# arpg/ba

Measured on AMD Instinct MI355X. Metric: Gauss-Newton iterations/sec, higher is better.
Workload: dtype f64; 1 GPU; BASELINE.json configs[3]: 10000 poses / 1000000 landmarks / 10000000 reprojection residuals, pinhole, LmSize=1, PoseSize=6, Gauss-Newton (no dogleg), 2 anchor poses inactive; poses=10000, landmarks=1000000, residuals=10000000, reduced_system_n=59988, driver=phase calls of the C-ABI (include/ba_hip.h), parallelism=single GPU

## Files before the change

ba_amd/csrc/chol_kernels.h:

```cpp
#pragma once
#include "engine.h"

namespace bae {

void launch_panel_chain(const CholSwitches& sw, hipStream_t s, double* dA, uint32_t ld, uint32_t nblk, uint32_t J,
                        uint32_t Jend, double* dsgn, double* opbuf, int* colneg, int* flags, const uint8_t* nz,
                        const uint32_t* rl = nullptr, uint32_t rl_n = 0, bool rl_square = false, bool sq = false);
void launch_step_update(hipStream_t s, dim3 grid, double* dA, uint32_t ld, uint32_t nblk, uint32_t c0, uint32_t kb0,
                        uint32_t kb1, double* dsgn, double* opbuf, int* colneg, int* flags, const uint8_t* nz,
                        const uint32_t* rl);
void launch_rect128(const CholSwitches& sw, const Rect128Shape& r, hipStream_t s, double* dA, uint32_t ld, uint32_t nblk,
                    uint32_t c0, uint32_t ncols, uint32_t kb0, uint32_t kb1, const double* dsgn, const int* colneg,
                    const uint8_t* nz, const OwnMap& own);
void launch_bulk_update(const CholSwitches& sw, Engine* e, hipStream_t s, double* dA, uint32_t ld, uint32_t nblk,
                        uint32_t a_end, uint32_t J, uint32_t Jend, const double* dsgn, const int* colneg,
                        const uint8_t* nz, bool full, const OwnMap& own, const uint2* pairs = nullptr,
                        uint32_t npairs = 0);
void launch_linvT(hipStream_t s, uint32_t nblk, const double* opbuf, const double* dsgn, double* linvT);
void launch_backward(hipStream_t s, double* dA, uint32_t ld, uint32_t nblk, const double* linvT, double* dx,
                     const uint8_t* nz, uint32_t lo = 0, uint32_t hi = 0xffffffffu);
int setup_status_block(Engine* e, const double* dA, uint32_t ld, hipStream_t s0);

}
```

ba_amd/csrc/chol_launch.h:

```cpp
#pragma once
#include <stdint.h>
#include <stdlib.h>
#include <string.h>

#include <algorithm>

namespace bae {

static const uint32_t kTile = 64;
static const uint32_t kPacketStride = 40 * 64;
static const uint32_t kKin = 4;

struct CholSwitches {
  bool no128 = false;
  bool no_lookahead = false;
  bool bulk_full = false;
  bool dense = false;
  bool no_dist_solve = false;
  uint32_t sbl = 3;
  uint32_t rect_min_rows = 128;
  uint32_t bulk_full_m = 128;
  bool c_rmw = false;
  uint32_t kout = 4;
  uint32_t left_min_tiles = 512;
  bool square = false;
  uint32_t sq_w = kKin;
  const char* dist_layout = nullptr;
  bool dense_scatter = false;
  const char* trace_file = nullptr;
};

inline uint32_t parse_kout(const char* v, uint32_t nblk) {
  const uint32_t k = v ? (uint32_t)atoi(v) : 0;
  return k ? k : (nblk >= 400 ? 16u : nblk >= 256 ? 8u : 4u);
}
inline void parse_process_switches(CholSwitches* sw, const char* no128, const char* no_lookahead, const char* bulk_full,
                                   const char* dense, const char* no_dist_solve, const char* sbl,
                                   const char* bulk_full_m, const char* c_rmw = nullptr) {
  sw->no128 = no128 != nullptr;
  sw->no_lookahead = no_lookahead != nullptr;
  sw->bulk_full = bulk_full != nullptr;
  sw->dense = dense != nullptr;
  sw->no_dist_solve = no_dist_solve != nullptr;
  sw->sbl = sbl ? (uint32_t)atoi(sbl) : 3u;
  sw->rect_min_rows = bulk_full_m ? (uint32_t)std::max(16, atoi(bulk_full_m)) : 128u;
  sw->bulk_full_m = bulk_full_m ? (uint32_t)atoi(bulk_full_m) : 128u;
  sw->c_rmw = c_rmw != nullptr;
}
inline void parse_call_switches(CholSwitches* sw, uint32_t nblk, const char* kout, const char* left_min_tiles,
                                const char* square, const char* sq_w, const char* dist_layout,
                                const char* dense_scatter, const char* trace_file) {
  sw->kout = parse_kout(kout, nblk);
  sw->left_min_tiles = left_min_tiles ? (uint32_t)std::max(1, atoi(left_min_tiles)) : 512u;
  sw->square = nblk < 512 && square && atoi(square) != 0;
  sw->sq_w = sq_w ? std::min(4u, std::max(1u, (uint32_t)atoi(sq_w))) : kKin;
  sw->dist_layout = dist_layout;
  sw->dense_scatter = dense_scatter != nullptr;
  sw->trace_file = trace_file;
}

inline const CholSwitches& chol_process_switches() {
  static const CholSwitches once = [] {
    CholSwitches sw;
    parse_process_switches(&sw, getenv("BA_HIP_NO128"), getenv("BA_HIP_NO_LOOKAHEAD"), getenv("BA_HIP_BULK_FULL"),
                           getenv("BA_HIP_DENSE"), getenv("BA_HIP_NO_DIST_SOLVE"), getenv("BA_HIP_SBL"),
                           getenv("BA_HIP_BULK_FULL_M"), getenv("BA_HIP_C_RMW"));
    return sw;
  }();
  return once;
}
inline CholSwitches chol_switches(uint32_t nblk) {
  CholSwitches sw = chol_process_switches();
  parse_call_switches(&sw, nblk, getenv("BA_HIP_KOUT"), getenv("BA_HIP_LEFT_MIN_TILES"), getenv("BA_HIP_SQUARE"),
                      getenv("BA_HIP_SQ_W"), getenv("BA_HIP_DIST_LAYOUT"), getenv("BA_HIP_DENSE_SCATTER"),
                      getenv("BA_HIP_TRACE_FILE"));
  return sw;
}
inline uint32_t kout_from_env(uint32_t nblk) { return parse_kout(getenv("BA_HIP_KOUT"), nblk); }

struct ChainShape { bool left; uint32_t kin; };
inline ChainShape chain_shape(uint32_t nblk, const CholSwitches& sw) {
  const bool left = nblk >= sw.left_min_tiles;
  return {left, left ? 2 * kKin : kKin};
}

struct Rect128Shape { bool use128; uint32_t m2, rect_cols, nrow64, grid; };
enum RectRule { kRectSingle, kRectDist };
inline Rect128Shape rect128_shape(RectRule rule, uint32_t nblk, uint32_t c0, uint32_t ncols, uint32_t G,
                                  const CholSwitches& sw) {
  const uint32_t r0 = c0 + ncols, m = nblk - r0;
  const bool single = r0 + sw.rect_min_rows <= nblk;
  const bool dist = m >= 16 && G % 2u == 0;
  Rect128Shape r = {!sw.no128 && (rule == kRectSingle ? single : dist) && ncols % 2u == 0 && c0 % 2u == 0, 0, 0, 0, 0};
  if (!r.use128) return r;
  r.m2 = m / 2;
  r.rect_cols = ncols / 2;
  r.nrow64 = (ncols * (1 + (m & 1u)) + 7) / 8 * 8;
  r.grid = r.nrow64 + r.m2 * r.rect_cols;
  return r;
}

enum BulkKernel { kBulkU128, kBulkU128List, kBulkU2Full, kBulkU2Capped };
struct BulkShape { BulkKernel kernel; uint32_t grid, nrow64, m2, sbl; int swzf; };
inline BulkShape bulk_shape(uint32_t nblk, uint32_t a_end, bool full, uint32_t own_n, uint32_t own_G, bool have_pairs,
                            uint32_t npairs, const CholSwitches& sw) {
  const uint32_t m = nblk - a_end;
  if (full && !sw.no128 && m >= 16 && (a_end % 2u) == 0 && (own_n <= 1 || own_G % 2u == 0)) {
    const uint32_t m2 = m / 2, sbl2 = 2, sbe2 = 1u << sbl2;
    const uint32_t nsr = (m2 + sbe2 - 1) / sbe2, nsb = nsr * (nsr + 1) / 2;
    const uint32_t nrow64 = (m * (1 + (m & 1u)) + 7) / 8 * 8;
    if (have_pairs && own_n > 1 && a_end % own_G == 0)
      return {kBulkU128List, nrow64 + npairs * (own_G / 2) * (own_G / 2), nrow64, m2, sbl2, 0};
    return {kBulkU128, nrow64 + ((nsb + 7) / 8) * 8 * sbe2 * sbe2, nrow64, m2, sbl2, 0};
  }
  const uint32_t sbe = 1u << sw.sbl;
  const uint32_t nsr = (m + 1 + sbe - 1) / sbe, nsb = nsr * (nsr + 1) / 2;
  return {full ? kBulkU2Full : kBulkU2Capped, ((nsb + 7) / 8) * 8 * sbe * sbe, 0, 0, sw.sbl, 1 | (int)(sw.sbl << 8)};
}

struct FactorWork {
  size_t dsgn, linvT, opbuf, colneg, total;
  explicit FactorWork(uint32_t nblk)
      : dsgn(0), linvT((size_t)nblk * kTile), opbuf(linvT + (size_t)nblk * kTile * kTile),
        colneg(opbuf + (size_t)nblk * kPacketStride), total(colneg + (nblk + 1) / 2) {}
};

inline uint64_t dist_plan_key(uint64_t nzL_version, uint32_t kout, bool pat, const char* layout, bool dense_scatter) {
  static const char* const names[] = {"auto", "tri", "grid", "col", "row"};
  uint64_t lay = layout && *layout ? 5 : 0;
  for (uint64_t i = 0; i < 5 && lay == 5; ++i)
    if (!strcmp(layout, names[i])) lay = i;
  return (pat ? nzL_version : 0) << 24 | (uint64_t)std::min(kout, 0xffffu) << 8 | lay << 2 |
         (dense_scatter ? 2u : 0u) | (pat ? 1u : 0u);
}

}
```

ba_amd/csrc/engine.h:

```cpp
#pragma once
#include <hip/hip_runtime.h>
#include <stdint.h>
#include <atomic>
#include <string>
#include <utility>
#include <vector>

#include "../../include/ba_hip.h"
#include "structure.h"
#include "ordering.h"
#include "selinv.h"
#include "marg.h"
#include "pcg.h"
#include "dist_plan.h"
#include "lifecycle.h"
#include "chol_launch.h"

namespace bae {

inline std::atomic<int64_t> g_device_bytes_live{0};
template <typename T>
struct DBuf {
  T* p = nullptr;
  size_t n = 0;
  DBuf() = default;
  DBuf(const DBuf&) = delete;
  DBuf& operator=(const DBuf&) = delete;
  DBuf(DBuf&& o) noexcept : p(o.p), n(o.n) { o.p = nullptr; o.n = 0; }
  DBuf& operator=(DBuf&& o) noexcept {
    if (this != &o) { release(); p = o.p; n = o.n; o.p = nullptr; o.n = 0; }
    return *this;
  }
  ~DBuf() { release(); }
  hipError_t alloc(size_t count) {
    if (count <= n && p) return hipSuccess;
    release();
    if (count == 0) { n = 0; return hipSuccess; }
    hipError_t err = hipMalloc((void**)&p, count * sizeof(T));
    if (err == hipSuccess) { n = count; g_device_bytes_live += (int64_t)bytes(); }
    return err;
  }
  void release() {
    if (p) { (void)hipFree(p); g_device_bytes_live -= (int64_t)bytes(); }
    p = nullptr;
    n = 0;
  }
  size_t bytes() const { return n * sizeof(T); }
};

static const int kRt = 12;
static const int kCamRec = 37;
static const int kPoseState = 16;
static const int kRow = 6;

struct Structure : Lists {
  uint32_t n_pp_entries = 0;
};

struct Engine {
  int lm_dim = 1, pose_dim = 6, device = 0;
  int calib_dim = 0;
  bool calib_tvs = false;
  std::vector<double> cam_params_prev;
  std::vector<double> cam_w_prev;
  bool has_fov = false;
  DBuf<double> lm_zref;
  hipStream_t stream = nullptr;
  hipStream_t stream2 = nullptr;
  std::vector<hipEvent_t> ev_panel, ev_bulk;
  hipEvent_t ev_imu_start = nullptr, ev_imu_done = nullptr;
  hipEvent_t ev_fork = nullptr, ev_join = nullptr;
  bool imu_early_pending = false;
  bool own_stream = false;
  std::string err;
  ba_hip_options opt;
  Problem prob;
  Structure st;
  Held held;
  int cur = 0;
  ba_hip_timers timers;
// ... 19 lines not shown
  DBuf<double> pose_cam;
  const double* pose_cam_ptr() const { return prob.pose_cam_params.empty() ? nullptr : pose_cam.p; }
  DBuf<int32_t> pose_opt, lm_opt;
  DBuf<uint16_t> pose_mask;
  DBuf<uint16_t> pose_mask_lin;
  uint64_t mask_version = 0, lin_mask_version = 0;
  const uint16_t* lin_pose_mask() const { return mask_version == lin_mask_version ? pose_mask.p : pose_mask_lin.p; }
  DBuf<uint32_t> lm_ref_pose, lm_ref_cam;
  DBuf<uint32_t> lm_ptr;
  DBuf<double> obs_z;
  DBuf<uint32_t> obs_pose, obs_cam, obs_lm, obs_rid;
  DBuf<double> obs_w0;
  DBuf<uint8_t> obs_cond;
  DBuf<uint2> wave_rng;
  DBuf<uint32_t> tile_ptr;
  DBuf<uint2> tile_ref;
  DBuf<uint32_t> tile_order;
  DBuf<uint4> tile_desc;
  uint32_t n_tile_order = 0;
  uint64_t tile_order_version = ~0ull;
  uint64_t tile_order_plan = ~0ull;
  int dbg_assemble_variant = 5;
  int dbg_host_structure = 0;
  int dbg_linearize_variant = 0;
  int dbg_tile_order = 0;
  int dbg_imu_wave = -1;
  int dbg_all_tiles = 0;
  DBuf<uint2> pair_ent;
  DBuf<uint32_t> pose_ptr, pose_mid;
  DBuf<uint32_t> pose_ent;
  DBuf<uint8_t> nzL;
  std::vector<uint8_t> nzL_host;
  uint64_t nzL_version = 0;
  std::vector<uint8_t> nzS_host;
  struct Dist {
    uint64_t key = ~0ull;
    DistPlan plan;
    DistTables tab;
    DBuf<uint32_t> tiles;
    DBuf<uint2> pairs;
    DBuf<uint32_t> square_rows;
    DBuf<uint32_t> dense_rows;
    DBuf<uint4> send_rects, recv_rects;
    DBuf<double> msg;
    DBuf<double> usend, urecv;
    DBuf<double> ssend, srecv;
    DBuf<double> back;
    hipStream_t stream3 = nullptr;
    hipStream_t stream4 = nullptr;
    void* comm2 = nullptr;
    std::vector<hipEvent_t> ev;
  } dist;
  void sharding_changed() { held.sharding_changed(); dist.key = ~0ull; }
  std::string dist_layout_name;
  ba_hip_comm_stats cstats = {};
  DBuf<double> packed;

  DBuf<uint8_t> pose_active;
  DBuf<uint32_t> un_pose; DBuf<double> un_t, un_cov_inv, un_scale; DBuf<uint8_t> un_rot;
  DBuf<uint32_t> bin_p1, bin_p2; DBuf<double> bin_t, bin_cov_inv, bin_cov_inv_sqrt, bin_w;
  DBuf<uint8_t> bin_rot;
  DBuf<uint32_t> imu_p1, imu_p2, imu_ptr; DBuf<double> imu_meas, imu_consts, imu_cov_inv;
  bool imu_cov_once = false;
  DBuf<double> imu_frozen;
  DBuf<double> imu_steps;
  DBuf<uint8_t> imu_cov_done;
// ... 220 lines not shown
int launch_end_solve(Engine* e);
int launch_residual_vectors(Engine* e, double* d_r2);
int launch_residuals(Engine* e, int mode);
int launch_landmarks(Engine* e, double c_huber, int use_robust);
int launch_gather_S(Engine* e);
int launch_pack_lower(Engine* e, int unpack);
size_t packed_lower_count(uint32_t n_pad);
int launch_backsub(Engine* e);
int launch_compose_step(Engine* e, double coef_rhs, double coef_gn, double* norms2_host);
int launch_apply_step(Engine* e);
int launch_dogleg(Engine* e, int gn_available, double* h7, bool skip_jrhs);
int select_kth(Engine* e, const double* d_values, uint32_t n_local, uint64_t k, double* out);
int sum_partials(Engine* e, uint32_t nparts, uint32_t ncomp, double* host_out, bool cross_shard = true);
void defer_begin(Engine* e);
int defer_flush(Engine* e);
struct DeferScope {
  Engine* e;
  bool flushed = false;
  explicit DeferScope(Engine* eng) : e(eng) { defer_begin(e); }
  DeferScope(const DeferScope&) = delete;
  DeferScope& operator=(const DeferScope&) = delete;
  int flush() { flushed = true; return defer_flush(e); }
  ~DeferScope() {
    if (flushed) return;
    e->defer_active = false;
    e->defer_n = 0;
  }
};
int launch_imu_early(Engine* e, double c_huber_proj);
int launch_posepose_build(Engine* e, double c_huber_proj, double* h3);
int launch_posepose_eval(Engine* e, double* h3);
int launch_posepose_jrhs(Engine* e, double* out);
int cholesky_solve(Engine* e, double* dA, uint32_t n, uint32_t ld, double* dx, int* status,
                   const uint8_t* nz_tiles);
int factor_tile_pattern(Engine* e);
uint32_t choose_kout(uint32_t nblk);
bool dist_solve_enabled(const Engine* e);
int dist_reduce_scatter_S(Engine* e);
int launch_imu_residual_vectors(Engine* e, double* d_r15);
int build_tile_order(Engine* e);
int build_tile_desc(Engine* e);
int dist_assembly_tiles(Engine* e, std::vector<uint8_t>* need);
int build_lists_device(Engine* e, const std::function<void(const char*)>& stage);
int order_poses(Engine* e, std::vector<uint64_t>* proj_edges, double device_ms);
bool ordering_wants_graph(const Engine* e);
int dist_broadcast(Engine* e, double* buf, size_t count, int root, hipStream_t s);
struct DistXfer { double* buf; size_t count; int peer; bool send; };
int dist_exchange(Engine* e, const std::vector<DistXfer>& x, bool side, hipStream_t s);
int dist_allreduce_stream(Engine* e, double* buf, size_t count, hipStream_t s);
void comm_release(Engine* e);
int check_solve_residual(Engine* e, const double* dS, const double* dx, const double* db, double* out2);
int cholesky_solve_dist(Engine* e, double* dA, uint32_t ld, double* dx, int* status, const uint8_t* nz);
int trailing_marginals(Engine* e, const double* dA, uint32_t ld, uint32_t first, uint32_t K, double* cov);
int marginals_compute(Engine* e);
int marginals_gather(Engine* e, uint32_t n, const std::vector<uint32_t>& ra, const std::vector<uint32_t>& rb, int Da,
                     int Db, double* out);
int marginals_landmarks(Engine* e, uint32_t n, const uint32_t* ids, double* out);
void marginals_release(Engine* e);
int leverages_run(Engine* e, uint32_t n, const uint32_t* ids, double* out);
int pose_pose_leverages_run(Engine* e, int kind, uint32_t n, const uint32_t* ids, double* cov, double* info, double* lev);
int jointcov_run(Engine* e, const std::vector<uint32_t>& sel, const std::vector<uint32_t>& lms, double* out);
void jointcov_release(Engine* e);
struct JointPlan;
struct SubstTables {
  const uint4 *chunks, *rows;
  const uint32_t *src, *pos;
};
// ... 34 lines not shown
```

ba_amd/csrc/engine.hip:

```cpp
#include "entry.h"
#include <chrono>
#include <functional>
#include <memory>
#include <thread>

#include <algorithm>
#include <cmath>
#include <cstdlib>
#include <cstring>
#include <numeric>

#include "dmath.h"
#include "factorsolve.h"
#include "dpose.h"

namespace bae {

int Engine::fail(hipError_t e, const char* what) {
  err = std::string(what) + ": " + hipGetErrorString(e);
  return -(int)(e == hipSuccess ? 1 : e);
}
void Engine::prof_collect() {
  auto drain = [](std::vector<std::pair<hipEvent_t, hipEvent_t>>& v, double& ms, uint32_t& n) {
    for (auto& p : v) {
// ... 972 lines not shown
    if (!e->held.nzL_valid && (rc = factor_tile_pattern(e))) return rc;
    const bool rebuild = e->pcg_plan_version != e->nzL_version || e->pcg_plan.nt != st.ld / 64 || e->pcg_blk.size() != (size_t)2 * st.ld;
    if (rebuild) {
      build_pcg_plan(e->nzS_host, st.ld / 64, e->pcg_plan);
      pcg_row_blocks(st.np, (uint32_t)e->pose_dim, st.K, st.ld, e->pcg_blk, e->pcg_blocks);
      e->pcg_plan_version = e->nzL_version;
      e->pcg_coarse_built = 0;
    }
    if (e->pcg_opt.coarse_aggregate && e->pcg_coarse_built != e->pcg_opt.coarse_aggregate) {
      const uint32_t D = (uint32_t)e->pose_dim;
      std::vector<uint32_t> nat(st.ld, kPcgNone);
      uint32_t a = 0;
      for (uint32_t p = 0; p < st.P; ++p)
        if (st.pose_opt[p] >= 0) {
          for (uint32_t d = 0; d < D; ++d) nat[(size_t)st.pose_opt[p] * D + d] = a * D + d;
          ++a;
        }
      for (uint32_t k = 0; k < st.K; ++k) nat[st.np + k] = st.Pact * D + k;
      build_pcg_coarse(e->pcg_plan, nat, st.Pact, D, st.K, e->pcg_opt.coarse_aggregate);
      e->pcg_coarse_built = e->pcg_opt.coarse_aggregate;
    }
    if ((rc = pcg_solve_device(e, e->A.p, st.n, st.ld, e->rhs_sc.p, e->pcg_plan, e->nzS_host, e->pcg_blk, e->pcg_blocks, rebuild,
                               e->pcg_opt, e->gn_p.p, &e->pcg_stats, &status))) return rc;
    e->held.solved_by_pcg();
  } else if (st.n > 0 && !skip) {
    if (e->opt.keep_reduced_system) {
      BAE_HIP(e->A_keep.alloc((size_t)st.ld * st.ld));
      BAE_HIP(hipMemcpyAsync(e->A_keep.p, e->A.p, (size_t)st.ld * st.ld * sizeof(double),
                             hipMemcpyDeviceToDevice, e->stream));
    }
    if (!e->held.nzL_valid && (rc = factor_tile_pattern(e))) return rc;
    if (dist_solve_enabled(e)) {
      if ((rc = cholesky_solve_dist(e, e->A.p, st.ld, e->gn_p.p, &status, e->nzL.p))) return rc;
    } else if ((rc = cholesky_solve(e, e->A.p, st.n, st.ld, e->gn_p.p, &status, e->nzL.p))) return rc;
    e->held.solved_directly();
  }
  e->timers.solve = t.stop_ms();
  EventTimer tb(e);
  if ((rc = launch_backsub(e))) return rc;
  e->timers.back_substitution = tb.stop_ms();
  return status ? BA_HIP_FACTORIZATION_ERROR : 0;
}

int ba_hip_dogleg_terms(ba_hip_engine* h, int gn_available, ba_hip_dogleg_scalars* out) {
  BA_ENTRY_FINAL(h);
  memset(out, 0, sizeof(*out));
  double* dh = e->dog_h;
  const bool reuse = gn_available && e->held.dog_jrhs_valid;
  DeferScope sums(e);
  int rc = launch_dogleg(e, gn_available, dh, reuse);
  if (!rc && !reuse) rc = launch_posepose_jrhs(e, dh + 7);
  if (!rc && !reuse) rc = launch_priors_jrhs(e, &e->prior_jrhs_h);
  if (!rc) rc = sums.flush();
  e->held.dogleg_sums(!rc);
  if (rc) return rc;
  out->rhs_p_sq = dh[0]; out->gn_p_sq = dh[1]; out->rhs_gn_p = dh[2];
  out->rhs_l_sq = dh[3]; out->gn_l_sq = dh[4]; out->rhs_gn_l = dh[5];
  out->j_rhs_sq = dh[6] + dh[7] + e->prior_jrhs_h;
  return e->st.K ? launch_calib_dogleg(e, gn_available, out) : 0;
}

int ba_hip_compose_step(ba_hip_engine* h, double coef_rhs, double coef_gn, ba_hip_step_norms* out) {
  BA_ENTRY_FINAL(h);
  double n2[2];
  DeferScope sums(e);
  int rc = launch_compose_step(e, coef_rhs, coef_gn, n2);
  if (!rc) rc = sums.flush();
// ... 369 lines not shown
```

ba_amd/csrc/engine_readers.hip:

```cpp
#include <algorithm>
#include <cmath>
#include <cstring>

#include "entry.h"
#include "factorsolve.h"

namespace bae {

static_assert(kRequestMaxBlock == kPcgMaxBlock, "block_ok of requests.h states the limit of pcg.h");

struct PaddedSystem {
  uint32_t ld = 0, nt = 0;
  std::vector<double> A;
  std::vector<uint8_t> nz;
};
static PaddedSystem pad_system(uint32_t n, const double* a_lower, const double* b, bool want_nz) {
  PaddedSystem s;
  const uint32_t ld = s.ld = std::max(((n + 63) / 64) * 64, 64u), nt = s.nt = ld / 64;
  s.A.assign((size_t)(ld + 1) * ld, 0.0);
  if (want_nz) s.nz.assign((size_t)nt * nt, 0);
  for (uint32_t r = 0; r < n; ++r)
    for (uint32_t c = 0; c <= r; ++c) {
      const double v = a_lower[(size_t)r * n + c];
      s.A[(size_t)r * ld + c] = v;
// ... 661 lines not shown
  const int rc = pcg_panel_solve_device(e, dA.p, n, ld, plan, sys.nz, blk, blocks, identity_rowmap(n, ld).data(), m, B, X, *o, &status);
  if (rc) return rc;
  e->held.pcg_run_finished(false);
  if (stats) *stats = e->pcgp_stats;
  return status ? BA_HIP_FACTORIZATION_ERROR : 0;
}

static int tile_factorise(Engine* e, const char* who, uint32_t n, const double* a_lower, const double* b,
                          const uint8_t* tile_map, PaddedSystem& sys, DBuf<double>& dA, DBuf<double>& dx, int* status) {
  sys = pad_system(n, a_lower, b, true);
  const uint32_t ld = sys.ld, nt = sys.nt;
  std::vector<uint8_t>& nz = sys.nz;
  if (tile_map) {
    for (uint32_t r = 0; r < n; ++r)
      for (uint32_t c = 0; c <= r; ++c)
        if (a_lower[(size_t)r * n + c] != 0.0 && r / 64 != c / 64 && !tile_map[(size_t)(r / 64) * nt + c / 64]) {
          e->err = std::string(who) + ": entry (" + std::to_string(r) + ", " + std::to_string(c) + ") is nonzero but tile (" +
                   std::to_string(r / 64) + ", " + std::to_string(c / 64) + ") is not in the tile map";
          return -1;
        }
    for (uint32_t i = 0; i < nt; ++i)
      for (uint32_t k = 0; k <= i; ++k) nz[(size_t)i * nt + k] |= tile_map[(size_t)i * nt + k] ? 1 : 0;
  }
  for (uint32_t i = 0; i < nt; ++i) nz[(size_t)i * nt + i] = 1;
  tile_symbolic_factor(nz, nt);
  DBuf<uint8_t> dnz;
  BAE_HIP(dA.alloc(sys.A.size()));
  BAE_HIP(dx.alloc(ld));
  BAE_HIP(dnz.alloc(nz.size()));
  BAE_HIP(e->flags.alloc(16));
  BAE_HIP(hipMemcpy(dA.p, sys.A.data(), sys.A.size() * 8, hipMemcpyHostToDevice));
  BAE_HIP(hipMemcpy(dnz.p, nz.data(), nz.size(), hipMemcpyHostToDevice));
  e->held.standalone_factorisation();
  int rc = cholesky_solve(e, dA.p, n, ld, dx.p, status, dnz.p);
  if (rc) return rc;
  BAE_HIP(hipDeviceSynchronize());
  return 0;
}
int ba_hip_tile_solve(ba_hip_engine* h, uint32_t n, const double* a_lower, const double* b, const uint8_t* tile_map,
                      double* x, uint8_t* nz_factor, double* factor, double* linvT, double* dsgn) {
  BA_ENTRY_DEVICE(h);
  if (!n || !a_lower || !b || !x) return e->fail_msg("ba_hip_tile_solve: NULL or empty argument");
  PaddedSystem sys;
  DBuf<double> dA, dx;
  int status = 0;
  if (int rc = tile_factorise(e, "ba_hip_tile_solve", n, a_lower, b, tile_map, sys, dA, dx, &status)) return rc;
  const uint32_t ld = sys.ld, nt = sys.nt;
  if (nz_factor) std::copy(sys.nz.begin(), sys.nz.end(), nz_factor);
  hipError_t err = download_x(dx, n, x);
  if (err == hipSuccess && factor) err = hipMemcpy(factor, dA.p, (size_t)ld * ld * 8, hipMemcpyDeviceToHost);
  const FactorWork fw(nt);
  if (err == hipSuccess && dsgn) err = hipMemcpy(dsgn, e->invdiag.p + fw.dsgn, (size_t)ld * 8, hipMemcpyDeviceToHost);
  if (err == hipSuccess && linvT)
    err = hipMemcpy(linvT, e->invdiag.p + fw.linvT, (size_t)nt * 64 * 64 * 8, hipMemcpyDeviceToHost);
  if (err != hipSuccess) return e->fail(err, "hipMemcpy");
  return status ? BA_HIP_FACTORIZATION_ERROR : 0;
}

int ba_hip_tile_factor_solve(ba_hip_engine* h, uint32_t n, const double* a_lower, const uint8_t* tile_map, uint32_t m,
                             const double* B, double* X) {
  BA_ENTRY_DEVICE(h);
  static const char* what = "ba_hip_tile_factor_solve";
  if (!n || !a_lower) return e->fail_msg("ba_hip_tile_factor_solve: NULL or empty argument");
  BA_ASK(columns_ok(what, m, BA_HIP_FACTOR_SOLVE_MAX_COLUMNS, "BA_HIP_FACTOR_SOLVE_MAX_COLUMNS"));
  if (!B || !X) return e->fail_msg("ba_hip_tile_factor_solve: NULL argument");
  PaddedSystem sys;
  DBuf<double> dA, dx;
// ... 11 lines not shown
```

ba_amd/csrc/hostcheck.cpp:

```cpp
#include <vector>
#include "dmath.h"
using namespace bad;

static Rt rt_from7(const double* p) {
  Rt t;
  t.R = quat_to_rot(p[3], p[4], p[5], p[6]);
  t.t = v3(p[0], p[1], p[2]);
  return t;
}

static double g_hostcheck_fov_w = 0.0;
extern "C" void ba_hostcheck_set_fov(double w) { g_hostcheck_fov_w = w; }
static Cam cam_from4(const double* cam4) {
  Cam c = {cam4[0], cam4[1], cam4[2], cam4[3], g_hostcheck_fov_w, g_hostcheck_fov_w != 0.0 ? 1 : 0};
  return c;
}

static int g_hostcheck_variant = 1;
extern "C" void ba_hostcheck_set_variant(int v) { g_hostcheck_variant = v; }

extern "C" void ba_hostcheck_proj_jacobians(int lm_dim, const double* cam4, const double* z,
                                            const double* x, const double* t_wp_m7,
                                            const double* t_vs_m7, const double* t_wp_r7,
                                            const double* t_vs_r7, int same_pose, double* r2,
// ... 807 lines not shown
      const int64_t v[15] = {sw.no128, sw.no_lookahead, sw.bulk_full, sw.dense, sw.no_dist_solve, sw.sbl,
                             sw.rect_min_rows, sw.bulk_full_m, sw.kout, sw.left_min_tiles, sw.square, sw.sq_w,
                             sw.dist_layout != nullptr, sw.dense_scatter, sw.trace_file != nullptr};
      std::copy(v, v + 15, out);
    } else if (op == 1) {
      const int64_t* a = in + (size_t)i * 2;
      sw.left_min_tiles = (uint32_t)a[1];
      const ChainShape c = chain_shape((uint32_t)a[0], sw);
      out[(size_t)i * 2] = c.left; out[(size_t)i * 2 + 1] = c.kin;
    } else if (op == 2) {
      const int64_t* a = in + (size_t)i * 7;
      sw.no128 = a[5] != 0; sw.rect_min_rows = (uint32_t)a[6];
      const Rect128Shape r = rect128_shape(a[0] ? kRectDist : kRectSingle, (uint32_t)a[1], (uint32_t)a[2], (uint32_t)a[3],
                                           (uint32_t)a[4], sw);
      const int64_t v[5] = {r.use128, r.m2, r.rect_cols, r.nrow64, r.grid};
      std::copy(v, v + 5, out + (size_t)i * 5);
    } else if (op == 3) {
      const int64_t* a = in + (size_t)i * 9;
      sw.no128 = a[7] != 0; sw.sbl = (uint32_t)a[8];
      const BulkShape b = bulk_shape((uint32_t)a[0], (uint32_t)a[1], a[2] != 0, (uint32_t)a[3], (uint32_t)a[4], a[5] != 0,
                                     (uint32_t)a[6], sw);
      const int64_t v[6] = {b.kernel, b.grid, b.nrow64, b.m2, b.sbl, b.swzf};
      std::copy(v, v + 6, out + (size_t)i * 6);
    } else if (op == 4) {
      const FactorWork fw((uint32_t)in[i]);
      const int64_t v[6] = {(int64_t)fw.dsgn, (int64_t)fw.linvT, (int64_t)fw.opbuf, (int64_t)fw.colneg, (int64_t)fw.total,
                            kPacketStride};
      std::copy(v, v + 6, out + (size_t)i * 6);
    } else if (op == 5) {
      out[0] = (int64_t)dist_plan_key((uint64_t)in[0], (uint32_t)in[1], in[2] != 0, str[0], in[3] != 0);
    } else if (op == 7) {
      parse_process_switches(&sw, nullptr, nullptr, nullptr, nullptr, nullptr, nullptr, nullptr, str[0]);
      out[0] = sw.c_rmw;
    } else {
      return -1;
    }
  }
  return 0;
}

#include "dist_plan.h"

extern "C" int64_t ba_hostcheck_dist_tables(int op, const uint32_t* hdr, const char* layout, const uint8_t* nzL, const uint8_t* nz2,
                                            const uint64_t* bits, const int64_t* arg, int64_t* out, uint64_t cap, char* msg,
                                            uint32_t msg_cap) {
  using namespace bae;
  const uint32_t nblk = hdr[0], N = hdr[2], rank = hdr[3];
  OwnMap map;
  if (!build_own_map(N, layout, hdr[1], &map, nullptr)) return -2;
  map.rank = rank;
  const DistPlan pl = build_dist_plan(nblk, map, nzL, N == 1);
  std::vector<int64_t> v;
  auto put = [&](const auto& list) { v.insert(v.end(), list.begin(), list.end()); };
  if (op == 0) {
    const DistOwnedPairs o = dist_owned_pairs(pl);
    v.push_back((int64_t)o.pairs.size());
    put(o.pair_first);
    for (const DistPair& p : o.pairs) { v.push_back(p.bi); v.push_back(p.bc); }
  } else if (op == 1) {
    put(dist_square_rows(pl));
  } else if (op == 2) {
    const DistDenseRows d = dist_dense_scatter_rows(pl, nz2);
    v.push_back((int64_t)d.chunk); v.push_back((int64_t)d.rows.size());
    put(d.off); put(d.chunk_off); put(d.rows);
  } else if (op == 3) {
    const size_t words = dist_pattern_words(nblk);
    static_assert(sizeof(unsigned long long) == sizeof(uint64_t), "pattern words");
    const unsigned long long* all = reinterpret_cast<const unsigned long long*>(bits);
    const DistSparseRects t = arg[0] < 0 ? dist_sparse_rects(pl, rank, all, words)
                                         : dist_sparse_rects(pl, rank, all, words, (uint64_t)arg[0]);
    v.push_back(!t.refused.empty()); v.push_back((int64_t)t.send.size()); v.push_back((int64_t)t.recv.size());
// ... 160 lines not shown
```

ba_amd/csrc/k_chol.hip:

```cpp
#include "engine.h"
#include "chol_kernels.h"
#include <cstdlib>
#include <algorithm>
#include <vector>

namespace bae {

static const int NB = 64;
static const int LDT = NB + 2;

typedef double double4_t __attribute__((ext_vector_type(4)));

__device__ __forceinline__ double readlane_f64(double v, int lane) {
  int lo = __double2loint(v), hi = __double2hiint(v);
  lo = __builtin_amdgcn_readlane(lo, lane);
  hi = __builtin_amdgcn_readlane(hi, lane);
  return __hiloint2double(hi, lo);
}

static const int LDM = 18;

static const int KC2 = 16;
#ifndef BAE_LDK2
#define BAE_LDK2 (KC2 + 2)
#endif
static const int LDK2 = BAE_LDK2;

__device__ __forceinline__ void update_tile_fast(double* __restrict__ A, uint32_t ld, uint32_t i, uint32_t c,
                                                 uint32_t kb0, uint64_t mask, double (*X)[NB][LDK2],
                                                 double (*Y)[NB][LDK2]) {
  const int tid = threadIdx.x, wave = tid >> 6, lane = tid & 63;
  const int li = lane & 15, lk = lane >> 4;
  const int rb = 32 * (wave >> 1), cb = 32 * (wave & 1);
  double* Aic = A + ((size_t)i * NB) * ld + (size_t)c * NB;
  double4_t acc[2][2];
#pragma unroll
// ... 1407 lines not shown
                    uint32_t c0, uint32_t ncols, uint32_t kb0, uint32_t kb1, const double* dsgn, const int* colneg,
                    const uint8_t* nz, const OwnMap& own) {
  auto kernel = sw.c_rmw ? k_update128<true, false, true> : k_update128<true>;
  hipLaunchKernelGGL(kernel, dim3(r.grid), dim3(256), 0, s, dA, ld, nblk, c0, r.m2, kb0, kb1, dsgn, colneg,
                     0u, nz, own, r.nrow64, c0 + ncols, r.rect_cols);
}
static void launch_next_panel_update(const CholSwitches& sw, hipStream_t s, double* dA, uint32_t ld, uint32_t nblk,
                                     uint32_t c0, uint32_t ncols, uint32_t kb0, uint32_t kb1, double* dsgn,
                                     double* opbuf, int* colneg, int* flags, const uint8_t* nz, bool factor = true) {
  auto step_update = factor ? k_step_update<true> : k_step_update<false>;
  const Rect128Shape r = rect128_shape(kRectSingle, nblk, c0, ncols, 1, sw);
  if (r.use128) {
    hipLaunchKernelGGL(step_update, dim3(ncols, ncols), dim3(256), 0, s, dA, ld, nblk, c0, kb0, kb1, dsgn, opbuf,
                       colneg, flags, nz, c0 + ncols, (const uint32_t*)nullptr);
    launch_rect128(sw, r, s, dA, ld, nblk, c0, ncols, kb0, kb1, dsgn, colneg, nz, own_map_single());
    return;
  }
  hipLaunchKernelGGL(step_update, dim3(nblk - c0 + 1, ncols), dim3(256), 0, s, dA, ld, nblk, c0, kb0, kb1, dsgn,
                     opbuf, colneg, flags, nz, nblk + 1u, (const uint32_t*)nullptr);
}

void launch_step_update(hipStream_t s, dim3 grid, double* dA, uint32_t ld, uint32_t nblk, uint32_t c0, uint32_t kb0,
                        uint32_t kb1, double* dsgn, double* opbuf, int* colneg, int* flags, const uint8_t* nz,
                        const uint32_t* rl) {
  hipLaunchKernelGGL(k_step_update<true>, grid, dim3(256), 0, s, dA, ld, nblk, c0, kb0, kb1, dsgn, opbuf, colneg, flags, nz,
                     nblk + 1u, rl);
}
void launch_linvT(hipStream_t s, uint32_t nblk, const double* opbuf, const double* dsgn, double* linvT) {
  hipLaunchKernelGGL(k_linvT, dim3(nblk), dim3(256), 0, s, opbuf, dsgn, linvT);
}

void launch_bulk_update(const CholSwitches& sw, Engine* e, hipStream_t s, double* dA, uint32_t ld, uint32_t nblk,
                        uint32_t a_end, uint32_t J, uint32_t Jend, const double* dsgn, const int* colneg,
                        const uint8_t* nz, bool full, const OwnMap& own, const uint2* pairs, uint32_t npairs) {
  const BulkShape b = bulk_shape(nblk, a_end, full, own.n, own.G, pairs != nullptr, npairs, sw);
  const dim3 grid(b.grid), wg(256);
  e->prof_begin(e->ev_syrk, s);
  switch (b.kernel) {
    case kBulkU128List: {
      OwnMap ol = own;
      ol.pairs_lo = (uint32_t)(reinterpret_cast<unsigned long long>(pairs) & 0xffffffffull);
      ol.pairs_hi = (uint32_t)(reinterpret_cast<unsigned long long>(pairs) >> 32);
      auto kernel = sw.c_rmw ? k_update128<false, true, true> : k_update128<false, true>;
      hipLaunchKernelGGL(kernel, grid, wg, 0, s, dA, ld, nblk, a_end, b.m2, J, Jend, dsgn, colneg, b.sbl, nz, ol,
                         b.nrow64, a_end, 0u);
      break;
    }
    case kBulkU128: {
      auto kernel = sw.c_rmw ? k_update128<false, false, true> : k_update128<false>;
      hipLaunchKernelGGL(kernel, grid, wg, 0, s, dA, ld, nblk, a_end, b.m2, J, Jend, dsgn, colneg, b.sbl, nz, own,
                         b.nrow64, a_end, 0u);
      break;
    }
    case kBulkU2Full:
      hipLaunchKernelGGL(k_update2<false>, grid, wg, 0, s, dA, ld, nblk, a_end, J, Jend, dsgn, colneg, b.swzf, nz, own);
      break;
    case kBulkU2Capped:
      hipLaunchKernelGGL(k_update2<true>, grid, wg, 0, s, dA, ld, nblk, a_end, J, Jend, dsgn, colneg, b.swzf, nz, own);
      break;
  }
  e->prof_end(e->ev_syrk, s);
}

__global__ void k_pivot_floor(uint32_t n_pad, uint32_t ld, const double* __restrict__ A, double tol,
                              double* __restrict__ out) {
  const uint32_t j = blockIdx.x * blockDim.x + threadIdx.x;
  if (j < n_pad) out[j] = tol * fabs(A[(size_t)j * ld + j]);
}

int setup_status_block(Engine* e, const double* dA, uint32_t ld, hipStream_t s0) {
  BAE_HIP(hipMemsetAsync(e->flags.p, 0, 4 * sizeof(int), s0));
// ... 45 lines not shown
      cov[(size_t)r * K + c] = s;
    }
  return 0;
}

#ifdef BAE_TIME128
static unsigned long long* t128_dev = nullptr;
static int time128_begin(Engine* e, const CholSwitches& sw) {
  if (!sw.trace_file) return 0;
  if (!t128_dev) {
    BAE_HIP(hipMalloc(&t128_dev, (size_t)T128_CAP * T128_REC * sizeof(unsigned long long)));
    BAE_HIP(hipMemcpyToSymbol(HIP_SYMBOL(g_t128_buf), &t128_dev, sizeof(t128_dev)));
  }
  const unsigned int zero = 0;
  BAE_HIP(hipMemcpyToSymbol(HIP_SYMBOL(g_t128_n), &zero, sizeof(zero)));
  return 0;
}
static int time128_write(Engine* e, const CholSwitches& sw) {
  if (!t128_dev || !sw.trace_file) return 0;
  BAE_HIP(hipDeviceSynchronize());
  unsigned int n = 0;
  BAE_HIP(hipMemcpyFromSymbol(&n, HIP_SYMBOL(g_t128_n), sizeof(n)));
  n = std::min(n, T128_CAP);
  std::vector<unsigned long long> rec((size_t)n * T128_REC);
  if (n) BAE_HIP(hipMemcpy(rec.data(), t128_dev, rec.size() * sizeof(unsigned long long), hipMemcpyDeviceToHost));
  if (FILE* f = fopen(sw.trace_file, "wb")) {
    fwrite(rec.data(), sizeof(unsigned long long), rec.size(), f);
    fclose(f);
  }
  return 0;
}
#endif

int cholesky_solve(Engine* e, double* dA, uint32_t n, uint32_t ld, double* dx, int* status,
                   const uint8_t* nz) {
  (void)n;
  const uint32_t nblk = ld / NB;
  const CholSwitches sw = chol_switches(nblk);
  const FactorWork fw(nblk);
  BAE_HIP(e->invdiag.alloc(fw.total));
  double* dsgn = e->invdiag.p + fw.dsgn;
  double* linvT = e->invdiag.p + fw.linvT;
  double* opbuf = e->invdiag.p + fw.opbuf;
  int* colneg = reinterpret_cast<int*>(e->invdiag.p + fw.colneg);
  hipStream_t s0 = e->stream, s1 = sw.no_lookahead ? e->stream : e->stream2;
  const uint32_t KOUT = sw.kout;
  const uint32_t npanels = (nblk + KOUT - 1) / KOUT;
  while (e->ev_panel.size() < npanels) {
    hipEvent_t a, b;
    BAE_HIP(hipEventCreateWithFlags(&a, hipEventDisableTiming));
    BAE_HIP(hipEventCreateWithFlags(&b, hipEventDisableTiming));
    e->ev_panel.push_back(a);
    e->ev_bulk.push_back(b);
  }
  { const int src = setup_status_block(e, dA, ld, s0); if (src) return src; }
#ifdef BAE_TIME128
  { const int trc = time128_begin(e, sw); if (trc) return trc; }
#endif
  const bool sq = sw.square;
  if (sq) {
    if (!e->square_attr_set) {
      BAE_HIP(hipFuncSetAttribute(reinterpret_cast<const void*>(k_square), hipFuncAttributeMaxDynamicSharedMemorySize,
                                  (int)sizeof(SquareLds)));
      BAE_HIP(hipFuncSetAttribute(reinterpret_cast<const void*>(k_rowpanel), hipFuncAttributeMaxDynamicSharedMemorySize,
                                  (int)sizeof(RowPanelLds)));
      e->square_attr_set = true;
    }
  } else {
    hipLaunchKernelGGL(k_step_update<true>, dim3(1, 1), dim3(256), 0, s0, dA, ld, nblk, 0u, 0u, 0u, dsgn, opbuf,
                       colneg, e->flags.p, nz, nblk + 1u, (const uint32_t*)nullptr);
  }
  int prev_bulk = -1;
  uint32_t pj = 0;
  for (uint32_t J = 0; J < nblk; J += KOUT, ++pj) {
    const uint32_t Jend = J + KOUT < nblk ? J + KOUT : nblk;
    launch_panel_chain(sw, s0, dA, ld, nblk, J, Jend, dsgn, opbuf, colneg, e->flags.p, nz, nullptr, 0, false, sq);
    if (Jend >= nblk) break;
    BAE_HIP(hipEventRecord(e->ev_panel[pj], s0));
    const uint32_t a_end = Jend + KOUT < nblk ? Jend + KOUT : nblk;
    if (prev_bulk >= 0) BAE_HIP(hipStreamWaitEvent(s0, e->ev_bulk[prev_bulk], 0));
    launch_next_panel_update(sw, s0, dA, ld, nblk, Jend, a_end - Jend, J, Jend, dsgn, opbuf, colneg, e->flags.p, nz, !sq);
    if (a_end < nblk) {
      BAE_HIP(hipStreamWaitEvent(s1, e->ev_panel[pj], 0));
      const uint32_t m = nblk - a_end;
      launch_bulk_update(sw, e, s1, dA, ld, nblk, a_end, J, Jend, dsgn, colneg, nz,
                         sw.no_lookahead || sw.bulk_full || m >= sw.bulk_full_m, own_map_single());
      BAE_HIP(hipEventRecord(e->ev_bulk[pj], s1));
      prev_bulk = (int)pj;
      if (e->profiling) {
        const bool pat = nz && e->nzL_host.size() == (size_t)nblk * nblk;
        e->kstats.syrk_flops += bulk_update_tile_products(own_map_single(), 0, nblk, a_end, J, Jend,
                                                          pat ? e->nzL_host.data() : nullptr) * 2.0 * NB * NB * NB;
      }
    }
  }
  BAE_HIP(hipGetLastError());
  hipLaunchKernelGGL(k_linvT, dim3(nblk), dim3(256), 0, s0, (const double*)opbuf, (const double*)dsgn,
                       linvT);
  launch_backward(s0, dA, ld, nblk, (const double*)linvT, dx, nz);
  BAE_HIP(hipGetLastError());
  int st = 0;
  BAE_HIP(hipMemcpyAsync(&st, e->flags.p, sizeof(int), hipMemcpyDeviceToHost, s0));
  BAE_HIP(hipStreamSynchronize(s0));
  *status = st;
#ifdef BAE_TIME128
  return time128_write(e, sw);
#endif
  return 0;
}

}
```

Baseline: 1.794 iterations/sec.

## Launch bulk trailing update over precomputed nonzero block lists

Builds host-side lists of the nonzero 128x128 tile pairs in each bulk trailing update, using the factor's sparsity pattern. The lists are spread evenly across 8 XCD slots and cached on the device, keyed by pattern version. The bulk update kernel then launches only over those listed blocks instead of a grid over every lower-triangle superblock, so empty blocks no longer cost a workgroup. In exchange it adds host list construction and an upload whenever the pattern changes, plus sentinel padding entries.

New measurement: 1.818 iterations/sec (median of 6 runs). 1.01x the previous value.

```diff
diff --git a/ba_amd/csrc/bulk_lists.h b/ba_amd/csrc/bulk_lists.h
--- /dev/null
+++ b/ba_amd/csrc/bulk_lists.h
@@ -0,0 +1,113 @@
+#pragma once
+#include <stdint.h>
+
+#include <vector>
+
+#include "chol_launch.h"
+
+namespace bae {
+
+static const uint32_t kBulkSentinel = 0xffffffffu;
+struct BulkEntry { uint32_t R, C; uint64_t mask; };
+
+static const size_t kBulkListBudgetBytes = (size_t)64 << 20;
+static const size_t kBulkListDeviceEntryBytes = 8;
+
+struct BulkLaunchList {
+  uint32_t a_end, J, Jend;
+  uint32_t first, len;
+  uint32_t blocks;
+  uint32_t xcd_blocks[8];
+};
+struct BulkLists {
+  bool built = false;
+  std::vector<BulkLaunchList> launches;
+  std::vector<BulkEntry> entries;
+  uint64_t total_blocks = 0;
+};
+
+inline bool bulk_launch_full(uint32_t nblk, uint32_t a_end, const CholSwitches& sw) {
+  return sw.no_lookahead || sw.bulk_full || nblk - a_end >= sw.bulk_full_m;
+}
+
+inline void build_bulk_launch_list(uint32_t nblk, uint32_t a_end, uint32_t J, uint32_t Jend, const uint8_t* nz,
+                                   BulkLists* out) {
+  const uint32_t m2 = (nblk - a_end) / 2, sbe = 4, nsr = (m2 + sbe - 1) / sbe;
+  const uint32_t ncol = Jend - J < 64u ? Jend - J : 64u;
+  std::vector<uint64_t> rowmask(m2, 0);
+  for (uint32_t R = 0; R < m2; ++R) {
+    const uint8_t* r0 = nz + (size_t)(a_end + 2 * R) * nblk + J;
+    const uint8_t* r1 = r0 + nblk;
+    uint64_t mk = 0;
+    for (uint32_t l = 0; l < ncol; ++l)
+      if (r0[l] | r1[l]) mk |= 1ull << l;
+    rowmask[R] = mk;
+  }
+  std::vector<BulkEntry> sub[8];
+  for (uint32_t sr = 0; sr < nsr; ++sr)
+    for (uint32_t sc = 0; sc <= sr; ++sc) {
+      BulkEntry blk[16];
+      uint32_t nb = 0;
+      for (uint32_t within = 0; within < sbe * sbe; ++within) {
+        const uint32_t R = sr * sbe + within / sbe, C = sc * sbe + within % sbe;
+        if (C > R || R >= m2) continue;
+        const uint64_t mk = rowmask[R] & rowmask[C];
+        if (mk) blk[nb++] = {R, C, mk};
+      }
+      if (!nb) continue;
+      uint32_t x = 0;
+      for (uint32_t y = 1; y < 8; ++y)
+        if (sub[y].size() < sub[x].size()) x = y;
+      sub[x].insert(sub[x].end(), blk, blk + nb);
+    }
+  BulkLaunchList l = {};
+  l.a_end = a_end; l.J = J; l.Jend = Jend;
+  l.first = (uint32_t)out->entries.size();
+  size_t longest = 0;
+  for (uint32_t x = 0; x < 8; ++x) {
+    l.xcd_blocks[x] = (uint32_t)sub[x].size();
+    l.blocks += l.xcd_blocks[x];
+    if (sub[x].size() > longest) longest = sub[x].size();
+  }
+  l.len = (uint32_t)(8 * longest);
+  const BulkEntry none = {kBulkSentinel, kBulkSentinel, 0};
+  for (size_t k = 0; k < longest; ++k)
+    for (uint32_t x = 0; x < 8; ++x) out->entries.push_back(k < sub[x].size() ? sub[x][k] : none);
+  out->total_blocks += l.blocks;
+  out->launches.push_back(l);
+}
+
+inline BulkLists build_bulk_lists(uint32_t nblk, uint32_t kout, const uint8_t* nz, const CholSwitches& sw,
+                                  size_t budget_bytes = kBulkListBudgetBytes) {
+  BulkLists out;
+  if (!nz || !kout || kout > 64u || sw.bulk_grid || sw.dense) return out;
+  for (uint32_t J = 0; J < nblk; J += kout) {
+    const uint32_t Jend = J + kout < nblk ? J + kout : nblk;
+    if (Jend >= nblk) break;
+    const uint32_t a_end = Jend + kout < nblk ? Jend + kout : nblk;
+    if (a_end >= nblk) continue;
+    if (bulk_shape(nblk, a_end, bulk_launch_full(nblk, a_end, sw), 1, 1, false, 0, sw).kernel != kBulkU128) continue;
+    build_bulk_launch_list(nblk, a_end, J, Jend, nz, &out);
+    if (out.entries.size() * kBulkListDeviceEntryBytes > budget_bytes) return BulkLists();
+  }
+  out.built = true;
+  return out;
+}
+
+struct BulkListsKey {
+  uint64_t nzL_version = ~0ull;
+  uint32_t nblk = 0, kout = 0, bulk_full_m = 0;
+  bool no128 = false, full_always = false;
+  bool operator==(const BulkListsKey& o) const {
+    return nzL_version == o.nzL_version && nblk == o.nblk && kout == o.kout && bulk_full_m == o.bulk_full_m &&
+           no128 == o.no128 && full_always == o.full_always;
+  }
+};
+inline BulkListsKey bulk_lists_key(uint64_t nzL_version, uint32_t nblk, const CholSwitches& sw) {
+  BulkListsKey k;
+  k.nzL_version = nzL_version; k.nblk = nblk; k.kout = sw.kout; k.bulk_full_m = sw.bulk_full_m;
+  k.no128 = sw.no128; k.full_always = sw.no_lookahead || sw.bulk_full;
+  return k;
+}
+
+}
diff --git a/ba_amd/csrc/chol_kernels.h b/ba_amd/csrc/chol_kernels.h
--- a/ba_amd/csrc/chol_kernels.h
+++ b/ba_amd/csrc/chol_kernels.h
@@ -15,7 +15,7 @@
 void launch_bulk_update(const CholSwitches& sw, Engine* e, hipStream_t s, double* dA, uint32_t ld, uint32_t nblk,
                         uint32_t a_end, uint32_t J, uint32_t Jend, const double* dsgn, const int* colneg,
                         const uint8_t* nz, bool full, const OwnMap& own, const uint2* pairs = nullptr,
-                        uint32_t npairs = 0);
+                        uint32_t npairs = 0, const uint2* blocks = nullptr, uint32_t nblocks = 0);
 void launch_linvT(hipStream_t s, uint32_t nblk, const double* opbuf, const double* dsgn, double* linvT);
 void launch_backward(hipStream_t s, double* dA, uint32_t ld, uint32_t nblk, const double* linvT, double* dx,
                      const uint8_t* nz, uint32_t lo = 0, uint32_t hi = 0xffffffffu);
diff --git a/ba_amd/csrc/chol_launch.h b/ba_amd/csrc/chol_launch.h
--- a/ba_amd/csrc/chol_launch.h
+++ b/ba_amd/csrc/chol_launch.h
@@ -21,6 +21,7 @@
   uint32_t rect_min_rows = 128;
   uint32_t bulk_full_m = 128;
   bool c_rmw = false;
+  bool bulk_grid = false;
   uint32_t kout = 4;
   uint32_t left_min_tiles = 512;
   bool square = false;
@@ -28,6 +29,7 @@
   const char* dist_layout = nullptr;
   bool dense_scatter = false;
   const char* trace_file = nullptr;
+  bool lists_report = false;
 };
 
 inline uint32_t parse_kout(const char* v, uint32_t nblk) {
@@ -36,7 +38,8 @@
 }
 inline void parse_process_switches(CholSwitches* sw, const char* no128, const char* no_lookahead, const char* bulk_full,
                                    const char* dense, const char* no_dist_solve, const char* sbl,
-                                   const char* bulk_full_m, const char* c_rmw = nullptr) {
+                                   const char* bulk_full_m, const char* c_rmw = nullptr,
+                                   const char* bulk_grid = nullptr) {
   sw->no128 = no128 != nullptr;
   sw->no_lookahead = no_lookahead != nullptr;
   sw->bulk_full = bulk_full != nullptr;
@@ -46,10 +49,12 @@
   sw->rect_min_rows = bulk_full_m ? (uint32_t)std::max(16, atoi(bulk_full_m)) : 128u;
   sw->bulk_full_m = bulk_full_m ? (uint32_t)atoi(bulk_full_m) : 128u;
   sw->c_rmw = c_rmw != nullptr;
+  sw->bulk_grid = bulk_grid != nullptr;
 }
 inline void parse_call_switches(CholSwitches* sw, uint32_t nblk, const char* kout, const char* left_min_tiles,
                                 const char* square, const char* sq_w, const char* dist_layout,
-                                const char* dense_scatter, const char* trace_file) {
+                                const char* dense_scatter, const char* trace_file,
+                                const char* lists_report = nullptr) {
   sw->kout = parse_kout(kout, nblk);
   sw->left_min_tiles = left_min_tiles ? (uint32_t)std::max(1, atoi(left_min_tiles)) : 512u;
   sw->square = nblk < 512 && square && atoi(square) != 0;
@@ -57,6 +62,7 @@
   sw->dist_layout = dist_layout;
   sw->dense_scatter = dense_scatter != nullptr;
   sw->trace_file = trace_file;
+  sw->lists_report = lists_report != nullptr;
 }
 
 inline const CholSwitches& chol_process_switches() {
@@ -64,7 +70,7 @@
     CholSwitches sw;
     parse_process_switches(&sw, getenv("BA_HIP_NO128"), getenv("BA_HIP_NO_LOOKAHEAD"), getenv("BA_HIP_BULK_FULL"),
                            getenv("BA_HIP_DENSE"), getenv("BA_HIP_NO_DIST_SOLVE"), getenv("BA_HIP_SBL"),
-                           getenv("BA_HIP_BULK_FULL_M"), getenv("BA_HIP_C_RMW"));
+                           getenv("BA_HIP_BULK_FULL_M"), getenv("BA_HIP_C_RMW"), getenv("BA_HIP_BULK_GRID"));
     return sw;
   }();
   return once;
@@ -73,7 +79,7 @@
   CholSwitches sw = chol_process_switches();
   parse_call_switches(&sw, nblk, getenv("BA_HIP_KOUT"), getenv("BA_HIP_LEFT_MIN_TILES"), getenv("BA_HIP_SQUARE"),
                       getenv("BA_HIP_SQ_W"), getenv("BA_HIP_DIST_LAYOUT"), getenv("BA_HIP_DENSE_SCATTER"),
-                      getenv("BA_HIP_TRACE_FILE"));
+                      getenv("BA_HIP_TRACE_FILE"), getenv("BA_HIP_BULK_LISTS_REPORT"));
   return sw;
 }
 inline uint32_t kout_from_env(uint32_t nblk) { return parse_kout(getenv("BA_HIP_KOUT"), nblk); }
@@ -100,10 +106,10 @@
   return r;
 }
 
-enum BulkKernel { kBulkU128, kBulkU128List, kBulkU2Full, kBulkU2Capped };
+enum BulkKernel { kBulkU128, kBulkU128List, kBulkU2Full, kBulkU2Capped, kBulkU128Blocks };
 struct BulkShape { BulkKernel kernel; uint32_t grid, nrow64, m2, sbl; int swzf; };
 inline BulkShape bulk_shape(uint32_t nblk, uint32_t a_end, bool full, uint32_t own_n, uint32_t own_G, bool have_pairs,
-                            uint32_t npairs, const CholSwitches& sw) {
+                            uint32_t npairs, const CholSwitches& sw, int64_t list_len = -1) {
   const uint32_t m = nblk - a_end;
   if (full && !sw.no128 && m >= 16 && (a_end % 2u) == 0 && (own_n <= 1 || own_G % 2u == 0)) {
     const uint32_t m2 = m / 2, sbl2 = 2, sbe2 = 1u << sbl2;
@@ -111,6 +117,8 @@
     const uint32_t nrow64 = (m * (1 + (m & 1u)) + 7) / 8 * 8;
     if (have_pairs && own_n > 1 && a_end % own_G == 0)
       return {kBulkU128List, nrow64 + npairs * (own_G / 2) * (own_G / 2), nrow64, m2, sbl2, 0};
+    if (list_len >= 0 && own_n <= 1 && !sw.bulk_grid)
+      return {kBulkU128Blocks, nrow64 + (uint32_t)list_len, nrow64, m2, sbl2, 0};
     return {kBulkU128, nrow64 + ((nsb + 7) / 8) * 8 * sbe2 * sbe2, nrow64, m2, sbl2, 0};
   }
   const uint32_t sbe = 1u << sw.sbl;
diff --git a/ba_amd/csrc/engine.h b/ba_amd/csrc/engine.h
--- a/ba_amd/csrc/engine.h
+++ b/ba_amd/csrc/engine.h
@@ -15,6 +15,7 @@
 #include "dist_plan.h"
 #include "lifecycle.h"
 #include "chol_launch.h"
+#include "bulk_lists.h"
 
 namespace bae {
 
@@ -46,6 +47,22 @@
     n = 0;
   }
   size_t bytes() const { return n * sizeof(T); }
+};
+
+struct BulkDeviceLists {
+  BulkListsKey key;
+  bool built = false;
+  std::vector<BulkLaunchList> launches;
+  DBuf<uint2> blocks;
+  uint64_t total_blocks = 0;
+  double build_ms = 0.0;
+  uint32_t builds = 0;
+  const BulkLaunchList* find(uint32_t a_end) const {
+    if (!built) return nullptr;
+    for (const BulkLaunchList& l : launches)
+      if (l.a_end == a_end) return &l;
+    return nullptr;
+  }
 };
 
 static const int kRt = 12;
@@ -131,6 +148,7 @@
   DBuf<uint8_t> nzL;
   std::vector<uint8_t> nzL_host;
   uint64_t nzL_version = 0;
+  BulkDeviceLists bulk_lists;
   std::vector<uint8_t> nzS_host;
   struct Dist {
     uint64_t key = ~0ull;
@@ -417,7 +435,8 @@
 int launch_posepose_eval(Engine* e, double* h3);
 int launch_posepose_jrhs(Engine* e, double* out);
 int cholesky_solve(Engine* e, double* dA, uint32_t n, uint32_t ld, double* dx, int* status,
-                   const uint8_t* nz_tiles);
+                   const uint8_t* nz_tiles, const BulkDeviceLists* lists = nullptr);
+int ensure_bulk_lists(Engine* e, uint32_t nblk, const uint8_t* nz_host, uint64_t version, BulkDeviceLists* lists);
 int factor_tile_pattern(Engine* e);
 uint32_t choose_kout(uint32_t nblk);
 bool dist_solve_enabled(const Engine* e);
diff --git a/ba_amd/csrc/engine.hip b/ba_amd/csrc/engine.hip
--- a/ba_amd/csrc/engine.hip
+++ b/ba_amd/csrc/engine.hip
@@ -1028,7 +1028,12 @@
     if (!e->held.nzL_valid && (rc = factor_tile_pattern(e))) return rc;
     if (dist_solve_enabled(e)) {
       if ((rc = cholesky_solve_dist(e, e->A.p, st.ld, e->gn_p.p, &status, e->nzL.p))) return rc;
-    } else if ((rc = cholesky_solve(e, e->A.p, st.n, st.ld, e->gn_p.p, &status, e->nzL.p))) return rc;
+    } else {
+      const uint32_t nt = st.ld / 64;
+      const bool pat = e->nzL_host.size() == (size_t)nt * nt;
+      if ((rc = ensure_bulk_lists(e, nt, pat ? e->nzL_host.data() : nullptr, e->nzL_version, &e->bulk_lists))) return rc;
+      if ((rc = cholesky_solve(e, e->A.p, st.n, st.ld, e->gn_p.p, &status, e->nzL.p, &e->bulk_lists))) return rc;
+    }
     e->held.solved_directly();
   }
   e->timers.solve = t.stop_ms();
diff --git a/ba_amd/csrc/engine_readers.hip b/ba_amd/csrc/engine_readers.hip
--- a/ba_amd/csrc/engine_readers.hip
+++ b/ba_amd/csrc/engine_readers.hip
@@ -717,7 +717,10 @@
   BAE_HIP(hipMemcpy(dA.p, sys.A.data(), sys.A.size() * 8, hipMemcpyHostToDevice));
   BAE_HIP(hipMemcpy(dnz.p, nz.data(), nz.size(), hipMemcpyHostToDevice));
   e->held.standalone_factorisation();
-  int rc = cholesky_solve(e, dA.p, n, ld, dx.p, status, dnz.p);
+  BulkDeviceLists lists;
+  int rc = ensure_bulk_lists(e, nt, nz.data(), ~0ull, &lists);
+  if (rc) return rc;
+  rc = cholesky_solve(e, dA.p, n, ld, dx.p, status, dnz.p, &lists);
   if (rc) return rc;
   BAE_HIP(hipDeviceSynchronize());
   return 0;
diff --git a/ba_amd/csrc/hostcheck.cpp b/ba_amd/csrc/hostcheck.cpp
--- a/ba_amd/csrc/hostcheck.cpp
+++ b/ba_amd/csrc/hostcheck.cpp
@@ -863,11 +863,40 @@
     } else if (op == 7) {
       parse_process_switches(&sw, nullptr, nullptr, nullptr, nullptr, nullptr, nullptr, nullptr, str[0]);
       out[0] = sw.c_rmw;
+    } else if (op == 8) {
+      parse_process_switches(&sw, nullptr, nullptr, nullptr, nullptr, nullptr, nullptr, nullptr, nullptr, str[0]);
+      out[0] = sw.bulk_grid;
+    } else if (op == 9) {
+      const int64_t* a = in + (size_t)i * 11;
+      sw.no128 = a[7] != 0; sw.sbl = (uint32_t)a[8]; sw.bulk_grid = a[10] != 0;
+      const BulkShape b = bulk_shape((uint32_t)a[0], (uint32_t)a[1], a[2] != 0, (uint32_t)a[3], (uint32_t)a[4], a[5] != 0,
+                                     (uint32_t)a[6], sw, a[9]);
+      const int64_t v[6] = {b.kernel, b.grid, b.nrow64, b.m2, b.sbl, b.swzf};
+      std::copy(v, v + 6, out + (size_t)i * 6);
     } else {
       return -1;
     }
   }
   return 0;
+}
+
+#include "bulk_lists.h"
+
+extern "C" int64_t ba_hostcheck_bulk_lists(const uint32_t* hdr, const uint8_t* nz, int64_t budget, int64_t* out, uint64_t cap) {
+  using namespace bae;
+  CholSwitches sw;
+  sw.no128 = hdr[2] != 0; sw.bulk_full_m = hdr[3]; sw.bulk_full = hdr[4] != 0; sw.bulk_grid = hdr[5] != 0; sw.dense = hdr[6] != 0;
+  const BulkLists l = budget < 0 ? build_bulk_lists(hdr[0], hdr[1], nz, sw) : build_bulk_lists(hdr[0], hdr[1], nz, sw, (size_t)budget);
+  const size_t need = 4 + 14 * l.launches.size() + 3 * l.entries.size();
+  if (need > cap) return -3;
+  int64_t* o = out;
+  *o++ = l.built; *o++ = (int64_t)l.launches.size(); *o++ = (int64_t)l.total_blocks; *o++ = (int64_t)l.entries.size();
+  for (const BulkLaunchList& b : l.launches) {
+    *o++ = b.a_end; *o++ = b.J; *o++ = b.Jend; *o++ = b.first; *o++ = b.len; *o++ = b.blocks;
+    for (uint32_t x = 0; x < 8; ++x) *o++ = b.xcd_blocks[x];
+  }
+  for (const BulkEntry& b : l.entries) { *o++ = b.R; *o++ = b.C; *o++ = (int64_t)b.mask; }
+  return (int64_t)need;
 }
 
 #include "dist_plan.h"
diff --git a/ba_amd/csrc/k_chol.hip b/ba_amd/csrc/k_chol.hip
--- a/ba_amd/csrc/k_chol.hip
+++ b/ba_amd/csrc/k_chol.hip
@@ -2,6 +2,7 @@
 #include "chol_kernels.h"
 #include <cstdlib>
 #include <algorithm>
+#include <chrono>
 #include <vector>
 
 namespace bae {
@@ -1475,11 +1476,23 @@
 
 void launch_bulk_update(const CholSwitches& sw, Engine* e, hipStream_t s, double* dA, uint32_t ld, uint32_t nblk,
                         uint32_t a_end, uint32_t J, uint32_t Jend, const double* dsgn, const int* colneg,
-                        const uint8_t* nz, bool full, const OwnMap& own, const uint2* pairs, uint32_t npairs) {
-  const BulkShape b = bulk_shape(nblk, a_end, full, own.n, own.G, pairs != nullptr, npairs, sw);
+                        const uint8_t* nz, bool full, const OwnMap& own, const uint2* pairs, uint32_t npairs,
+                        const uint2* blocks, uint32_t nblocks) {
+  const BulkShape b = bulk_shape(nblk, a_end, full, own.n, own.G, pairs != nullptr, npairs, sw,
+                                 blocks ? (int64_t)nblocks : -1);
   const dim3 grid(b.grid), wg(256);
   e->prof_begin(e->ev_syrk, s);
   switch (b.kernel) {
+    case kBulkU128Blocks: {
+      OwnMap ol = own;
+      ol.G = 2;
+      ol.pairs_lo = (uint32_t)(reinterpret_cast<unsigned long long>(blocks) & 0xffffffffull);
+      ol.pairs_hi = (uint32_t)(reinterpret_cast<unsigned long long>(blocks) >> 32);
+      auto kernel = sw.c_rmw ? k_update128<false, true, true> : k_update128<false, true>;
+      hipLaunchKernelGGL(kernel, grid, wg, 0, s, dA, ld, nblk, a_end, b.m2, J, Jend, dsgn, colneg, b.sbl, nz, ol,
+                         b.nrow64, a_end, 0u);
+      break;
+    }
     case kBulkU128List: {
       OwnMap ol = own;
       ol.pairs_lo = (uint32_t)(reinterpret_cast<unsigned long long>(pairs) & 0xffffffffull);
@@ -1591,8 +1604,43 @@
 }
 #endif
 
+int ensure_bulk_lists(Engine* e, uint32_t nblk, const uint8_t* nz_host, uint64_t version, BulkDeviceLists* L) {
+  const CholSwitches sw = chol_switches(nblk);
+  const BulkListsKey key = bulk_lists_key(version, nblk, sw);
+  if (version != ~0ull && L->key == key) return 0;
+  const auto t0 = std::chrono::steady_clock::now();
+  L->key = BulkListsKey();
+  L->built = false;
+  L->launches.clear();
+  L->total_blocks = 0;
+  const BulkLists lists = build_bulk_lists(nblk, sw.kout, nz_host, sw);
+  if (lists.built) {
+    std::vector<uint2> dev(lists.entries.size());
+    size_t at = 0;
+    for (const BulkLaunchList& l : lists.launches)
+      for (uint32_t k = 0; k < l.len; ++k, ++at) {
+        const BulkEntry& b = lists.entries[at];
+        dev[at] = b.R == kBulkSentinel ? make_uint2(kBulkSentinel, kBulkSentinel)
+                                       : make_uint2(l.a_end / 2 + b.R, l.a_end / 2 + b.C);
+      }
+    BAE_HIP(L->blocks.alloc(std::max<size_t>(dev.size(), 1)));
+    if (!dev.empty()) BAE_HIP(hipMemcpy(L->blocks.p, dev.data(), dev.size() * sizeof(uint2), hipMemcpyHostToDevice));
+  }
+  L->built = lists.built;
+  L->launches = lists.launches;
+  L->total_blocks = lists.total_blocks;
+  L->key = key;
+  L->build_ms = std::chrono::duration<double, std::milli>(std::chrono::steady_clock::now() - t0).count();
+  L->builds++;
+  if (sw.lists_report)
+    fprintf(stderr, "bulk lists: nblk %u kout %u built %d launches %zu blocks %llu entries %zu build_ms %.3f\n",
+            nblk, sw.kout, (int)L->built, L->launches.size(), (unsigned long long)L->total_blocks,
+            lists.entries.size(), L->build_ms);
+  return 0;
+}
+
 int cholesky_solve(Engine* e, double* dA, uint32_t n, uint32_t ld, double* dx, int* status,
-                   const uint8_t* nz) {
+                   const uint8_t* nz, const BulkDeviceLists* lists) {
   (void)n;
   const uint32_t nblk = ld / NB;
   const CholSwitches sw = chol_switches(nblk);
@@ -1641,9 +1689,10 @@
     launch_next_panel_update(sw, s0, dA, ld, nblk, Jend, a_end - Jend, J, Jend, dsgn, opbuf, colneg, e->flags.p, nz, !sq);
     if (a_end < nblk) {
       BAE_HIP(hipStreamWaitEvent(s1, e->ev_panel[pj], 0));
-      const uint32_t m = nblk - a_end;
-      launch_bulk_update(sw, e, s1, dA, ld, nblk, a_end, J, Jend, dsgn, colneg, nz,
-                         sw.no_lookahead || sw.bulk_full || m >= sw.bulk_full_m, own_map_single());
+      const BulkLaunchList* bl = nz && lists && lists->key.nblk == nblk ? lists->find(a_end) : nullptr;
+      if (bl && (bl->J != J || bl->Jend != Jend)) bl = nullptr;
+      launch_bulk_update(sw, e, s1, dA, ld, nblk, a_end, J, Jend, dsgn, colneg, nz, bulk_launch_full(nblk, a_end, sw),
+                         own_map_single(), nullptr, 0, bl ? lists->blocks.p + bl->first : nullptr, bl ? bl->len : 0);
       BAE_HIP(hipEventRecord(e->ev_bulk[pj], s1));
       prev_bulk = (int)pj;
       if (e->profiling) {
```
